# abelxiaoxing/ImageClassification

Hardware: AMD Instinct MI355X
Metric: images/sec (whole node) ResNet-50 bf16 224^2 training (higher is better)
Workload: dtype bf16; 1 GPU; resnet50 train step, synthetic 3x224x224, batch 256/GPU, AdamW, label smoothing 0.1, 1000 classes (BASELINE configs[1]); global_batch=256, parallelism=dp1

## Files before the change

imageclassification_amd/csrc/capi.hip:

```cpp
#include "capi_common.h"

bool g_prof_on = false;
std::vector<ProfRec> g_prof_recs;
std::vector<hipEvent_t> g_prof_pool;
hipEvent_t prof_event() {
  if (!g_prof_pool.empty()) { hipEvent_t e = g_prof_pool.back(); g_prof_pool.pop_back(); return e; }
  hipEvent_t e; (void)hipEventCreate(&e); return e;
}

extern "C" {

int icamd_abi_version(void) { return 6; }

int icamd_prof_enable(int on) { g_prof_on = on != 0; return ICAMD_OK; }
int icamd_prof_classes(void) { return PC_COUNT; }
int icamd_prof_collect(double* ms, long long* calls, double* bytes, double* flops, int n) {
  if (ms == nullptr || calls == nullptr || n < PC_COUNT) return ICAMD_ERR_BAD_ARG;
  for (auto& r : g_prof_recs) {
    (void)hipEventSynchronize(r.b);
    float t = 0.f;
    (void)hipEventElapsedTime(&t, r.a, r.b);
    ms[r.cls] += (double)t;
    calls[r.cls] += 1;
    if (bytes != nullptr) bytes[r.cls] += r.bytes;
    if (flops != nullptr) flops[r.cls] += r.flops;
    g_prof_pool.push_back(r.a);
    g_prof_pool.push_back(r.b);
  }
  g_prof_recs.clear();
  return ICAMD_OK;
}

int icamd_conv2d_stats_rows(const icamd_conv_desc* d) {
  if (!conv_desc_ok(d)) return 0;
  const long long M = (long long)d->N * d->OH * d->OW;
  return (int)((M + 127) / 128);
}

static int conv_fwd_impl(const icamd_conv_desc* d, const void* x, const void* w, void* y, const float* bias,
                         const void* addend, float* stats, int relu, void* stream, void* gelu_out = nullptr,
                         int gelu_inplace = 0) {
  if (!conv_desc_ok(d) || x == nullptr || w == nullptr || y == nullptr) return ICAMD_ERR_BAD_ARG;
  if ((long long)d->N * d->OH * d->OW >= (1ll << 31)) return ICAMD_ERR_UNSUPPORTED;
  if (d->KH == 3 && d->KW == 3 && d->stride == 1 && d->pad == 1 && addend == nullptr && gelu_out == nullptr &&
      !gelu_inplace && icamd_halo3x3_wanted(d->N, d->IH, d->IW, d->Cin, d->Cout)) {
    Halo3x3Params h;
    memset(&h, 0, sizeof(h));
    h.in = (const bf16_t*)x; h.wt = (const bf16_t*)w; h.out = (bf16_t*)y; h.bias = bias; h.stats = stats; h.relu = relu;
    h.N = d->N; h.H = d->IH; h.W = d->IW; h.C = d->Cin; h.Cout = d->Cout;
    return icamd_halo3x3_launch(h, (hipStream_t)stream);
  }
  const bool pw_gather = d->KH == 1 && d->KW == 1 && d->stride == 2 && d->pad == 0 && addend == nullptr;
  if (d->KH == 1 && d->KW == 1 && (d->stride == 1 || pw_gather) && d->pad == 0 && bias == nullptr && addend == nullptr && !relu &&
      gelu_out == nullptr && !gelu_inplace && icamd_pw_resident_wanted((long long)d->N * d->OH * d->OW, d->Cout, d->Cin)) {
    PwResidentParams g;
    memset(&g, 0, sizeof(g));
    g.A = (const bf16_t*)x; g.B = (const bf16_t*)w; g.out = (bf16_t*)y; g.stats = stats;
    g.M = d->N * d->OH * d->OW; g.N = d->Cout; g.K = d->Cin;
    if (pw_gather) { g.gat_oh = d->OH; g.gat_ow = d->OW; g.gat_ih = d->IH; g.gat_iw = d->IW; }
    return icamd_pw_resident_launch(g, (hipStream_t)stream);
  }
  if (d->KH == 1 && d->KW == 1 && (d->stride == 1 || pw_gather) && d->pad == 0 && (bias != nullptr || relu) && stats == nullptr &&
      gelu_out == nullptr && !gelu_inplace &&
      icamd_pw_resident_wanted((long long)d->N * d->OH * d->OW, d->Cout, d->Cin, addend != nullptr)) {
    PwResidentParams g;
    memset(&g, 0, sizeof(g));
    g.A = (const bf16_t*)x; g.B = (const bf16_t*)w; g.out = (bf16_t*)y; g.bias = bias; g.relu = relu;
    g.addend = (const bf16_t*)addend;
    g.M = d->N * d->OH * d->OW; g.N = d->Cout; g.K = d->Cin;
    if (pw_gather) { g.gat_oh = d->OH; g.gat_ow = d->OW; g.gat_ih = d->IH; g.gat_iw = d->IW; }
    return icamd_pw_resident_launch(g, (hipStream_t)stream);
  }
  if (d->KH == 1 && d->KW == 1 && d->stride == 1 && d->pad == 0 && addend == nullptr && !relu && stats == nullptr &&
      icamd_pw_resident_ext_wanted((long long)d->N * d->OH * d->OW, d->Cout, d->Cin)) {
    PwResidentParams g;
    memset(&g, 0, sizeof(g));
    g.A = (const bf16_t*)x; g.B = (const bf16_t*)w; g.out = (bf16_t*)y; g.bias = bias;
    g.gelu_out = (bf16_t*)gelu_out; g.gelu_inplace = gelu_inplace;
    g.M = d->N * d->OH * d->OW; g.N = d->Cout; g.K = d->Cin;
    return icamd_pw_resident_ext_launch(g, (hipStream_t)stream);
  }
  if (d->KH == 1 && d->KW == 1 && d->stride == 1 && d->pad == 0 &&
      icamd_gemm_nt_wanted((long long)d->N * d->OH * d->OW, d->Cout, d->Cin)) {
    GemmNtParams g;
    memset(&g, 0, sizeof(g));
    g.A = (const bf16_t*)x; g.B = (const bf16_t*)w; g.out = (bf16_t*)y; g.addend = (const bf16_t*)addend; g.bias = bias;
    g.stats = stats;
    g.M = d->N * d->OH * d->OW; g.N = d->Cout; g.K = d->Cin; g.relu = relu; g.gelu_out = (bf16_t*)gelu_out; g.gelu_inplace = gelu_inplace;
    return icamd_gemm_nt_launch(g, (hipStream_t)stream);
  }
  IgemmParams p;
  memset(&p, 0, sizeof(p));
  p.in = (const bf16_t*)x; p.wt = (const bf16_t*)w; p.out = (bf16_t*)y;
  p.addend = (const bf16_t*)addend; p.bias = bias; p.stats = stats; p.relu = relu; p.gelu_out = (bf16_t*)gelu_out; p.gelu_inplace = gelu_inplace;
  p.N = d->N; p.IH = d->IH; p.IW = d->IW; p.Cin = d->Cin;
  p.OH = d->OH; p.OW = d->OW; p.Cout = d->Cout;
  p.P = d->OH; p.Q = d->OW; p.M = d->N * d->OH * d->OW;
  p.ostr = 1; p.ooff_h = 0; p.ooff_w = 0; p.istr = d->stride;
  p.ntaps = d->KH * d->KW; p.Ktot = p.ntaps * d->Cin;
  p.KW = d->KW; p.pad = d->pad; p.tap_sign = 1; p.regular_taps = 1;
  if (p.ntaps <= ICAMD_MAX_TAPS)
    for (int r = 0; r < d->KH; ++r)
      for (int s = 0; s < d->KW; ++s) {
        const int t = r * d->KW + s;
        p.dh[t] = (short)(r - d->pad); p.dw[t] = (short)(s - d->pad); p.wtap[t] = (short)t;
      }
  return icamd_igemm_launch(p, (hipStream_t)stream);
}

int icamd_conv2d_fwd(const icamd_conv_desc* d, const void* x, const void* w, void* y, const float* bias,
                     const void* addend, float* stats, void* stream) {
  ProfScope _prof(PC_IGEMM_FWD, stream);
  const ConvWork cw = conv_work(d); _prof.work(cw.in + cw.out + 2 * cw.w + (addend ? cw.out : 0), cw.flops);
  return conv_fwd_impl(d, x, w, y, bias, addend, stats, 0, stream);
}

int icamd_conv2d_fwd_act(const icamd_conv_desc* d, const void* x, const void* w, void* y, const float* bias,
                         const void* addend, int relu, void* stream) {
  ProfScope _prof(PC_IGEMM_FWD, stream);
  const ConvWork cw = conv_work(d); _prof.work(cw.in + cw.out + 2 * cw.w + (addend ? cw.out : 0), cw.flops);
  return conv_fwd_impl(d, x, w, y, bias, addend, nullptr, relu ? 1 : 0, stream);
}

int icamd_conv2d_fwd_gelu(const icamd_conv_desc* d, const void* x, const void* w, void* z, void* a, const float* bias,
                          void* stream) {
  ProfScope _prof(PC_IGEMM_FWD, stream);
  const ConvWork cw = conv_work(d); _prof.work(cw.in + (z ? cw.out : 0) + cw.out + 2 * cw.w, cw.flops);
  if (a == nullptr) return ICAMD_ERR_BAD_ARG;
  if (z == nullptr) return conv_fwd_impl(d, x, w, a, bias, nullptr, nullptr, 0, stream, nullptr, 1);
  return conv_fwd_impl(d, x, w, z, bias, nullptr, nullptr, 0, stream, a);
}

static int dgrad_impl(const icamd_conv_desc* d, const void* dy, const void* w_t, void* dx, const void* addend,
                      const uint8_t* addend_bits, const icamd_bn_bwd_fuse* f, void* stream, const void* gelu_z = nullptr,
                      int addend_sub2 = 0) {
  if (!conv_desc_ok(d) || dy == nullptr || w_t == nullptr || dx == nullptr) return ICAMD_ERR_BAD_ARG;
  if (d->Cout % 8 != 0 || d->Cin % 8 != 0) return ICAMD_ERR_UNSUPPORTED;
  if ((long long)d->N * d->IH * d->IW >= (1ll << 31)) return ICAMD_ERR_UNSUPPORTED;
  const int st = d->stride;
  const bool pw_addend = icamd_pw_resident_mode() != 5;
  if (d->KH == 1 && d->KW == 1 && st == 1 && d->pad == 0 && f == nullptr && gelu_z == nullptr &&
      (addend == nullptr || pw_addend) && !(addend_bits != nullptr && addend_sub2) &&
      icamd_pw_resident_wanted((long long)d->N * d->IH * d->IW, d->Cin, d->Cout, addend != nullptr)) {
    PwResidentParams g;
    memset(&g, 0, sizeof(g));
    g.A = (const bf16_t*)dy; g.B = (const bf16_t*)w_t; g.out = (bf16_t*)dx; g.addend = (const bf16_t*)addend;
    g.addend_bits = addend_bits;
    g.M = d->N * d->IH * d->IW; g.N = d->Cin; g.K = d->Cout;
    if (addend_sub2) { g.sub2_h = d->IH; g.sub2_w = d->IW; }
    return icamd_pw_resident_launch(g, (hipStream_t)stream);
  }
  if (d->KH == 1 && d->KW == 1 && st == 1 && d->pad == 0 && f == nullptr && addend == nullptr &&
      icamd_pw_resident_ext_wanted((long long)d->N * d->IH * d->IW, d->Cin, d->Cout)) {
    PwResidentParams g;
    memset(&g, 0, sizeof(g));
    g.A = (const bf16_t*)dy; g.B = (const bf16_t*)w_t; g.out = (bf16_t*)dx; g.gelu_z = (const bf16_t*)gelu_z;
    g.M = d->N * d->IH * d->IW; g.N = d->Cin; g.K = d->Cout;
    return icamd_pw_resident_ext_launch(g, (hipStream_t)stream);
  }
  if (d->KH == 1 && d->KW == 1 && st == 1 && d->pad == 0 && f == nullptr && !(addend_bits != nullptr && addend_sub2) &&
      icamd_gemm_nt_wanted((long long)d->N * d->IH * d->IW, d->Cin, d->Cout)) {
    GemmNtParams g;
    memset(&g, 0, sizeof(g));
    g.A = (const bf16_t*)dy; g.B = (const bf16_t*)w_t; g.out = (bf16_t*)dx; g.addend = (const bf16_t*)addend;
    g.addend_bits = addend_bits;
    g.M = d->N * d->IH * d->IW; g.N = d->Cin; g.K = d->Cout; g.gelu_z = (const bf16_t*)gelu_z;
    if (addend_sub2) { g.sub2_h = d->IH; g.sub2_w = d->IW; }
    return icamd_gemm_nt_launch(g, (hipStream_t)stream);
  }
  if (d->KH == 3 && d->KW == 3 && st == 1 && d->pad == 1 && addend == nullptr && addend_bits == nullptr && f == nullptr &&
      gelu_z == nullptr && icamd_halo3x3_wanted(d->N, d->IH, d->IW, d->Cout, d->Cin)) {
    Halo3x3Params h;
    memset(&h, 0, sizeof(h));
    h.in = (const bf16_t*)dy; h.wt = (const bf16_t*)w_t; h.out = (bf16_t*)dx; h.flip = 1;
    h.N = d->N; h.H = d->IH; h.W = d->IW; h.C = d->Cout; h.Cout = d->Cin;
    return icamd_halo3x3_launch(h, (hipStream_t)stream);
  }
  float* partials = f ? f->partials : nullptr;
  for (int ph = 0; ph < st; ++ph)
    for (int pw = 0; pw < st; ++pw) {
      const int P = (d->IH - ph + st - 1) / st, Q = (d->IW - pw + st - 1) / st;
      if (P <= 0 || Q <= 0) continue;
      IgemmParams p;
      memset(&p, 0, sizeof(p));
      p.in = (const bf16_t*)dy; p.wt = (const bf16_t*)w_t; p.out = (bf16_t*)dx;
      p.addend = (const bf16_t*)addend;
      p.addend_bits = addend_bits;
      p.addend_sub2 = addend_sub2;
      p.gelu_z = (const bf16_t*)gelu_z;
      p.N = d->N; p.IH = d->OH; p.IW = d->OW; p.Cin = d->Cout;
      p.OH = d->IH; p.OW = d->IW; p.Cout = d->Cin;
      p.P = P; p.Q = Q; p.M = d->N * P * Q;
      p.ostr = st; p.ooff_h = ph; p.ooff_w = pw; p.istr = 1;
      p.Ktot = d->KH * d->KW * d->Cout;
      p.KW = d->KW; p.pad = d->pad; p.tap_sign = -1; p.regular_taps = (st == 1) ? 1 : 0;
      if (f != nullptr) {
        p.bnb_y = (const bf16_t*)f->y; p.bnb_mask = (const bf16_t*)f->mask_src;
        p.bnb_mean = f->mean; p.bnb_invstd = f->invstd; p.bnb_scale = f->scale; p.bnb_shift = f->shift;
        p.bnb_relu = f->relu; p.stats = partials;
        partials += (size_t)((p.M + 127) / 128) * 2 * d->Cin;
      }
      int nt = 0;
      for (int r = 0; r < d->KH; ++r) {
        const int eh = ph + d->pad - r;
        if (((eh % st) + st) % st != 0) continue;
        for (int s = 0; s < d->KW; ++s) {
          const int ew = pw + d->pad - s;
          if (((ew % st) + st) % st != 0) continue;
          if (nt < ICAMD_MAX_TAPS) { p.dh[nt] = (short)(eh / st); p.dw[nt] = (short)(ew / st); p.wtap[nt] = (short)(r * d->KW + s); }
          ++nt;
        }
      }
      p.ntaps = nt;
      const int rc = icamd_igemm_launch(p, (hipStream_t)stream);
      if (rc) return rc;
    }
  return ICAMD_OK;
}

int icamd_conv2d_dgrad(const icamd_conv_desc* d, const void* dy, const void* w_t, void* dx, const void* addend,
                       const uint8_t* addend_maskbits, void* stream) {
  ProfScope _prof(PC_IGEMM_DGRAD, stream);
  const ConvWork cw = conv_work(d); _prof.work(cw.out + cw.in + 2 * cw.w + (addend ? cw.in : 0) + (addend_maskbits ? cw.in / 16 : 0), cw.flops);
  if (addend_maskbits != nullptr && (addend == nullptr || d == nullptr || d->Cin % 64 != 0)) return ICAMD_ERR_BAD_ARG;
  return dgrad_impl(d, dy, w_t, dx, addend, addend_maskbits, nullptr, stream);
}

int icamd_conv2d_dgrad_sub2(const icamd_conv_desc* d, const void* dy, const void* w_t, void* dx, const void* addend_sub2,
                            void* stream) {
  ProfScope _prof(PC_IGEMM_DGRAD, stream);
  const ConvWork cw = conv_work(d); _prof.work(cw.out + cw.in + 2 * cw.w + cw.in / 4, cw.flops);
  if (addend_sub2 == nullptr) return ICAMD_ERR_BAD_ARG;
  return dgrad_impl(d, dy, w_t, dx, addend_sub2, nullptr, nullptr, stream, nullptr, 1);
}

int icamd_conv2d_dgrad_gelu(const icamd_conv_desc* d, const void* dy, const void* w_t, const void* z, void* dz,
                            void* stream) {
  ProfScope _prof(PC_IGEMM_DGRAD, stream);
  const ConvWork cw = conv_work(d); _prof.work(cw.out + 2 * cw.in + 2 * cw.w, cw.flops);
  if (z == nullptr) return ICAMD_ERR_BAD_ARG;
  return dgrad_impl(d, dy, w_t, dz, nullptr, nullptr, nullptr, stream, z);
}

int icamd_conv2d_dgrad_stats_rows(const icamd_conv_desc* d) {
  if (!conv_desc_ok(d)) return 0;
  int rows = 0;
  for (int ph = 0; ph < d->stride; ++ph)
    for (int pw = 0; pw < d->stride; ++pw) {
      const long long P = (d->IH - ph + d->stride - 1) / d->stride, Q = (d->IW - pw + d->stride - 1) / d->stride;
      if (P > 0 && Q > 0) rows += (int)((d->N * P * Q + 127) / 128);
    }
  return rows;
}

int icamd_conv2d_dgrad_bnbwd(const icamd_conv_desc* d, const void* dy, const void* w_t, void* g, const void* addend,
                             const icamd_bn_bwd_fuse* f, void* stream) {
  ProfScope _prof(PC_IGEMM_DGRAD, stream);
  const ConvWork cw = conv_work(d); _prof.work(cw.out + 2 * cw.in + 2 * cw.w + (addend ? cw.in : 0), cw.flops);
  if (f == nullptr || f->y == nullptr || f->mean == nullptr || f->invstd == nullptr || f->partials == nullptr)
// ... 89 lines not shown
```

imageclassification_amd/csrc/conv3x3_halo.hip:

```cpp
#ifndef ICAMD_C64_NT
#define ICAMD_C64_NT 0
#endif
#include "common.h"
#include "icamd_internal.h"
#include <cstdlib>

namespace {

template <int N> __device__ __forceinline__ void halo_wait_vmcnt() {
  static_assert(N >= 0 && N < 64, "vmcnt is a 6-bit field");
  asm volatile("s_waitcnt vmcnt(%0)" ::"n"(N) : "memory");
}

__device__ __forceinline__ int swzq(int blk) { return (0x78 >> (2 * blk)) & 3; }

template <int BN, int WN, int MFR, int LA, int NB, int KS, int WPS>
__global__ __launch_bounds__(256, WPS) void conv3x3_halo_kernel(const Halo3x3Params p) {
  constexpr int WM = 4 / WN;
  constexpr int BM = WM * MFR * 16;
  constexpr int NJ = BN / WN / 16;
  constexpr int A_SLOTS = 4 * LA * 8;
  constexpr int ZERO_SLOT = A_SLOTS - 1;
  constexpr int A_BYTES = A_SLOTS * 128;
  constexpr int B_STAGE = BN * KS * 2;
  constexpr int LB = BN * KS / 2048;
  static_assert(KS == 32 || KS == 64, "filter stage width");
  constexpr int RING = NB * B_STAGE;
  constexpr int EPI_BYTES = BM * BN * 2;
  constexpr int LDS_BYTES = (A_BYTES + RING > EPI_BYTES) ? A_BYTES + RING : EPI_BYTES;
  static_assert(NB >= 2 && NB <= 8 && (WN == 1 || WN == 2) && LB >= 1, "configuration");
  __shared__ __attribute__((aligned(16))) unsigned char smem[LDS_BYTES];
  unsigned char* const sA = smem;
  unsigned char* const sB = smem + A_BYTES;

  const int tid = threadIdx.x, lane = tid & 63;
  const int wave = __builtin_amdgcn_readfirstlane(tid >> 6);
  const int wm = wave % WM, wn = wave / WM;
  const int fr = lane & 15, fq = lane >> 4;

  const unsigned int nblk = gridDim.x;
  unsigned int L;
  {
    const unsigned int xcd = blockIdx.x & 7u, idx = blockIdx.x >> 3;
    const unsigned int q = nblk >> 3, r = nblk & 7u;
    L = (xcd < r ? xcd * (q + 1) : r * (q + 1) + (xcd - r) * q) + idx;
  }
  const int tile_m = L / p.ntiles_n, tile_n = L - tile_m * p.ntiles_n;
  const int m0 = tile_m * BM, n0 = tile_n * BN;
  const int W = p.W, C = p.C;
  const bf16_t* __restrict__ in = p.in;
  const bf16_t* __restrict__ wt = p.wt;
  const bf16_t* zero = (const bf16_t*)icamd_zero_page;

  const int a_slot_lane = lane >> 3;
  int b_src[LB];
#pragma unroll
  for (int j = 0; j < LB; ++j) {
    int row, lc;
    if constexpr (KS == 64) {
      row = (wave * LB + j) * 8 + (lane >> 3);
      lc = ((lane & 7) ^ ((row >> 1) & 7)) * 8;
    } else {
      row = (wave * LB + j) * 16 + (lane >> 2);
      lc = ((lane & 3) ^ swzq((row >> 2) & 3)) * 8;
    }
    const int co = n0 + row;
    b_src[j] = (co < p.Cout) ? co * 9 * C + lc : -1;
  }
  auto stage_a = [&](int slice) {
#pragma unroll
    for (int j = 0; j < LA; ++j) {
      const int slot = (wave * LA + j) * 8 + a_slot_lane;
      const int pix = m0 - (W + 1) + slot;
      const int lc = (((lane & 7) - slot) & 7) * 8;
      const bf16_t* src = (pix >= 0 && pix < p.M && slot != ZERO_SLOT) ? in + ((long long)pix * C + slice * 64 + lc) : zero;
      __builtin_amdgcn_global_load_lds(GPTR(src), LPTR(sA + (wave * LA + j) * 1024), 16, 0, 0);
    }
  };
  auto stage_b = [&](int slice, int tap, int kk, int slot) {
    const int wtap = p.flip ? 8 - tap : tap;
    const int off = wtap * C + slice * 64 + kk * 32;
#pragma unroll
    for (int j = 0; j < LB; ++j) {
      const bf16_t* src = b_src[j] >= 0 ? wt + (b_src[j] + off) : zero;
      __builtin_amdgcn_global_load_lds(GPTR(src), LPTR(sB + slot * B_STAGE + (wave * LB + j) * 1024), 16, 0, 0);
    }
  };

  int slot0[MFR];
  unsigned int vmask[MFR];
#pragma unroll
  for (int i = 0; i < MFR; ++i) {
    const int ml = wm * (BM / WM) + i * 16 + fr;
    const int m = m0 + ml;
    slot0[i] = ml + W + 1;
    unsigned int mk = 0;
    if (m < p.M) {
      const unsigned int n = fdiv((unsigned)m, p.divHW);
      const unsigned int rem = m - n * (p.H * W);
      const int h = (int)fdiv(rem, p.divW);
      const int w = (int)(rem - (unsigned)h * W);
#pragma unroll
      for (int t = 0; t < 9; ++t) {
        const int dh = t / 3 - 1, dw = t % 3 - 1;
        if ((unsigned)(h + dh) < (unsigned)p.H && (unsigned)(w + dw) < (unsigned)W) mk |= 1u << t;
      }
    }
    vmask[i] = mk;
  }
  f32x4 acc[NJ][MFR];
#pragma unroll
  for (int j = 0; j < NJ; ++j)
#pragma unroll
    for (int i = 0; i < MFR; ++i) acc[j][i] = f32x4{0.f, 0.f, 0.f, 0.f};

  const int nslices = C >> 6;
  constexpr int SPT = 64 / KS;
  const int nstages = nslices * 9 * SPT;
  stage_a(0);
  int issue_q = 0, issue_slice = 0, issue_tap = 0, issue_kk = 0, fill = 0;
  auto issue_b = [&]() {
    stage_b(issue_slice, issue_tap, issue_kk, fill);
    fill = fill == NB - 1 ? 0 : fill + 1;
    ++issue_q;
    if (++issue_kk == SPT) {
      issue_kk = 0;
      if (++issue_tap == 9) { issue_tap = 0; ++issue_slice; }
    }
  };
#pragma unroll
  for (int k = 0; k < NB - 1; ++k)
    if (issue_q < nstages) issue_b();

  const int b_row = wn * (BN / WN) + fr;
  const int b_frag = KS == 64 ? b_row * 128 : b_row * 64 + ((fq ^ swzq((fr >> 2) & 3)) << 4);
  const int bsw = (fr >> 1) & 7;
  int read = 0, q = 0;
  for (int slice = 0; slice < nslices; ++slice) {
#pragma unroll 1
    for (int tap = 0; tap < 9; ++tap) {
      const int trow = tap >= 6 ? 2 : (tap >= 3 ? 1 : 0);
      const int doff = (trow - 1) * W + (tap - 3 * trow - 1);
      const unsigned int tbit = 1u << tap;
      int aaddr[MFR];
#pragma unroll
      for (int i = 0; i < MFR; ++i) {
        const int sl = (vmask[i] & tbit) ? slot0[i] + doff : ZERO_SLOT;
        aaddr[i] = sl * 128 + (((fq + sl) & 7) << 4);
      }
#pragma unroll
      for (int st = 0; st < SPT; ++st, ++q) {
        {
          const int younger = issue_q - 1 - q;
          if (younger >= 4) halo_wait_vmcnt<4 * LB>();
          else if (younger == 3) halo_wait_vmcnt<3 * LB>();
          else if (younger == 2) halo_wait_vmcnt<2 * LB>();
          else if (younger == 1) halo_wait_vmcnt<LB>();
          else halo_wait_vmcnt<0>();
        }
        asm volatile("s_waitcnt lgkmcnt(0)" ::: "memory");
        __builtin_amdgcn_s_barrier();
        if (issue_q < nstages) issue_b();
        const unsigned char* sb = sB + read * B_STAGE + b_frag;
        read = read == NB - 1 ? 0 : read + 1;
#pragma unroll
        for (int kk = (KS == 64 ? 0 : st); kk < (KS == 64 ? 2 : st + 1); ++kk) {
          bf16x8 wf[NJ];
#pragma unroll
          for (int j = 0; j < NJ; ++j) {
            if constexpr (KS == 64) wf[j] = *(const bf16x8*)(sb + j * 2048 + (((kk * 4 + fq) ^ bsw) << 4));
            else wf[j] = *(const bf16x8*)(sb + j * 1024);
          }
#pragma unroll
          for (int i = 0; i < MFR; ++i) {
            const bf16x8 xf = *(const bf16x8*)(sA + (kk ? (aaddr[i] ^ 64) : aaddr[i]));
#pragma unroll
            for (int j = 0; j < NJ; ++j) acc[j][i] = __builtin_amdgcn_mfma_f32_16x16x32_bf16(wf[j], xf, acc[j][i], 0, 0, 0);
          }
        }
      }
    }
    if (slice + 1 < nslices) {
      asm volatile("s_waitcnt lgkmcnt(0)" ::: "memory");
      __builtin_amdgcn_s_barrier();
      stage_a(slice + 1);
      halo_wait_vmcnt<0>();
    }
  }
  __syncthreads();

  constexpr int ROWB = BN * 2, CPR = BN / 8;
#pragma unroll
  for (int j = 0; j < NJ; ++j) {
    const int cl = wn * (BN / WN) + j * 16 + 4 * fq;
    const int cg = n0 + cl;
    const int cgc = cg < p.Cout ? cg : 0;
    f32x4 b4 = {0.f, 0.f, 0.f, 0.f};
    if (p.bias != nullptr) b4 = *(const f32x4*)(p.bias + cgc);
#pragma unroll
    for (int i = 0; i < MFR; ++i) {
      const int ml = wm * (BM / WM) + i * 16 + fr;
      f32x4 v = acc[j][i] + b4;
      if (p.relu) {
#pragma unroll
        for (int e = 0; e < 4; ++e) v[e] = v[e] < 0.f ? 0.f : v[e];
      }
      u32x2 pk;
      pk[0] = pack_bf16x2(v[0], v[1]);
      pk[1] = pack_bf16x2(v[2], v[3]);
      const int slot = cl >> 2;
      *(u32x2*)(smem + ml * ROWB + ((((slot >> 1) ^ ml) & (CPR - 1)) << 4) + ((slot & 1) << 3)) = pk;
    }
  }
  __syncthreads();
  constexpr int RPP = 256 / CPR;
  constexpr int NPASS = BM / RPP;
  const int cp = tid & (CPR - 1), rg = tid / CPR;
  const int co = n0 + cp * 8;
  const bool co_ok = co < p.Cout;
  float s1[8], s2[8];
#pragma unroll
  for (int e = 0; e < 8; ++e) { s1[e] = 0.f; s2[e] = 0.f; }
#pragma unroll
  for (int ps = 0; ps < NPASS; ++ps) {
    const int ml = ps * RPP + rg;
    const int m = m0 + ml;
    const u32x4 o = *(const u32x4*)(smem + ml * ROWB + (((cp ^ ml) & (CPR - 1)) << 4));
    if (m < p.M && co_ok) {
      *(u32x4*)(p.out + (long long)m * p.Cout + co) = o;
      if (p.stats != nullptr) {
#pragma unroll
        for (int e = 0; e < 4; ++e) {
          const float lo = bf16_lo(o[e]), hi = bf16_hi(o[e]);
          s1[2 * e] += lo; s2[2 * e] += lo * lo;
          s1[2 * e + 1] += hi; s2[2 * e + 1] += hi * hi;
        }
      }
    }
  }
  if (p.stats != nullptr) {
    __syncthreads();
    float* red = (float*)smem;
#pragma unroll
    for (int e = 0; e < 8; ++e) {
      red[(rg * 2 + 0) * BN + cp * 8 + e] = s1[e];
      red[(rg * 2 + 1) * BN + cp * 8 + e] = s2[e];
    }
    __syncthreads();
    const int ntm = (p.M + BM - 1) / BM, nrows = (p.M + 127) / 128;
    for (int idx = tid; idx < 2 * BN; idx += 256) {
      const int which = idx / BN, c = idx - which * BN;
      float s = 0.f;
#pragma unroll 4
      for (int g = 0; g < RPP; ++g) s += red[(g * 2 + which) * BN + c];
      if (n0 + c < p.Cout) {
        p.stats[((long long)tile_m * 2 + which) * p.Cout + n0 + c] = s;
        if (ntm + tile_m < nrows) p.stats[((long long)(ntm + tile_m) * 2 + which) * p.Cout + n0 + c] = 0.f;
      }
    }
  }
}

template <bool ACT>
__global__ __launch_bounds__(256, 2) void conv3x3_c64_resident_kernel(const Halo3x3Params p, const int ntiles) {
  constexpr int BM = 128, LA = 8;
  constexpr int A_BYTES = 32 * LA * 128;
  constexpr int E_BYTES = 4 * 64 * 64;
  constexpr int ZERO_SLOT = 32 * LA - 1;
  __shared__ __attribute__((aligned(16))) unsigned char smem[2 * A_BYTES + E_BYTES];

  const int tid = threadIdx.x, lane = tid & 63;
  const int wave = __builtin_amdgcn_readfirstlane(tid >> 6);
  const int wm = wave & 1, wn = wave >> 1;
  const int fr = lane & 15, fq = lane >> 4;
  const int W = p.W, H = p.H;
  const bf16_t* __restrict__ in = p.in;
  const bf16_t* zero = (const bf16_t*)icamd_zero_page;
  unsigned char* const sE = smem + 2 * A_BYTES + wave * 4096;
  const unsigned lds_base = (unsigned)(uintptr_t)LPTR(smem);

  const int a_slot = wave * 8 + (lane >> 3);
  const int a_lc = (((lane & 7) - (lane >> 3)) & 7) * 8;
  const bool a_zero_lane = a_slot == 31;
  auto stage_a = [&](int m0, unsigned char* dst) {
    const int pix0 = m0 - (W + 1) + a_slot;
    const bf16_t* src0 = in + ((long long)pix0 * 64 + a_lc);
    if (m0 - (W + 1) >= 0 && m0 - (W + 1) + LA * 32 <= p.M) {
#pragma unroll
      for (int j = 0; j < LA; ++j) {
        const bf16_t* src = src0 + j * (32 * 64);
        if (j == LA - 1) src = a_zero_lane ? zero : src;
        __builtin_amdgcn_global_load_lds(GPTR(src), LPTR(dst + (j * 4 + wave) * 1024), 16, 0, ICAMD_C64_NT);
      }
    } else {
#pragma unroll
      for (int j = 0; j < LA; ++j) {
        const int pix = pix0 + j * 32;
        const bf16_t* src = (pix >= 0 && pix < p.M && !(j == LA - 1 && a_zero_lane)) ? src0 + j * (32 * 64) : zero;
        __builtin_amdgcn_global_load_lds(GPTR(src), LPTR(dst + (j * 4 + wave) * 1024), 16, 0, ICAMD_C64_NT);
      }
    }
  };

  int buf = 0;
  int tile = blockIdx.x;
  if (tile < ntiles) stage_a(tile * BM, smem);

  bf16x8 wf[18][2];
#pragma unroll
  for (int ks = 0; ks < 18; ++ks) {
    const int tap = ks >> 1;
// ... 93 lines not shown
      for (int i = 0; i < 4; ++i) {
        const int pl = i * 16 + fr;
        f32x4 v = acc[j][i];
        if constexpr (ACT) {
          v += b4;
          if (p.relu) {
#pragma unroll
            for (int e = 0; e < 4; ++e) v[e] = v[e] < 0.f ? 0.f : v[e];
          }
        }
        u32x2 pk;
        pk[0] = pack_bf16x2(v[0], v[1]);
        pk[1] = pack_bf16x2(v[2], v[3]);
        const int slot = j * 4 + fq;
        *(u32x2*)(sE + pl * 64 + ((((slot >> 1) ^ (pl >> 2)) & 3) << 4) + ((slot & 1) << 3)) = pk;
      }
    }
    {
      const int pl0 = lane >> 2;
      const int mrow = m0 + wm * 64 + pl0;
      bf16_t* orow = p.out + ((long long)mrow * 64 + wn * 32 + (lane & 3) * 8);
      const bool want_stats = p.stats != nullptr;
#pragma unroll
      for (int r = 0; r < 4; ++r) {
        const int pl = r * 16 + pl0;
        const u32x4 o = *(const u32x4*)(sE + pl * 64 + ((((lane & 3) ^ (pl >> 2)) & 3) << 4));
        if (mrow + r * 16 < p.M) {
          *(u32x4*)(orow + r * (16 * 64)) = o;
          if (want_stats) {
#pragma unroll
            for (int e = 0; e < 4; ++e) {
              const f32x2 v = {bf16_lo(o[e]), bf16_hi(o[e])};
              s1[e] += v;
              s2[e] = __builtin_elementwise_fma(v, v, s2[e]);
            }
          }
        }
      }
    }
  }

  if (p.stats != nullptr) {
    __syncthreads();
    float* red = (float*)smem;
    const int g = wm * 16 + (lane >> 2);
    const int c0 = wn * 32 + (lane & 3) * 8;
#pragma unroll
    for (int e = 0; e < 4; ++e) {
      red[(g * 2 + 0) * 64 + c0 + 2 * e] = s1[e][0];
      red[(g * 2 + 0) * 64 + c0 + 2 * e + 1] = s1[e][1];
      red[(g * 2 + 1) * 64 + c0 + 2 * e] = s2[e][0];
      red[(g * 2 + 1) * 64 + c0 + 2 * e + 1] = s2[e][1];
    }
    __syncthreads();
    if (tid < 128) {
      const int which = tid >> 6, c = tid & 63;
      float s = 0.f;
#pragma unroll 8
      for (int k = 0; k < 32; ++k) s += red[(k * 2 + which) * 64 + c];
      p.stats[((long long)blockIdx.x * 2 + which) * 64 + c] = s;
      const int nrows = (p.M + 127) / 128;
      for (int r = blockIdx.x + gridDim.x; r < nrows; r += gridDim.x) p.stats[((long long)r * 2 + which) * 64 + c] = 0.f;
    }
  }
}

int launch_resident_c64(const Halo3x3Params& p, hipStream_t stream) {
  const int ntiles = (p.M + 127) / 128;
  const int slots = 2 * icamd_num_cus();
  const int grid = ntiles < slots ? ntiles : slots;
  if (p.bias != nullptr || p.relu)
    hipLaunchKernelGGL((conv3x3_c64_resident_kernel<true>), dim3((unsigned)grid), dim3(256), 0, stream, p, ntiles);
  else
    hipLaunchKernelGGL((conv3x3_c64_resident_kernel<false>), dim3((unsigned)grid), dim3(256), 0, stream, p, ntiles);
  return icamd_launch_status();
}

template <int BN, int WN, int MFR, int LA, int NB, int KS, int WPS>
int launch_halo(const Halo3x3Params& p, hipStream_t stream) {
  constexpr int BM = (4 / WN) * MFR * 16;
  const int ntm = (p.M + BM - 1) / BM;
  hipLaunchKernelGGL((conv3x3_halo_kernel<BN, WN, MFR, LA, NB, KS, WPS>), dim3((unsigned)(ntm * p.ntiles_n)), dim3(256), 0,
                     stream, p);
  return icamd_launch_status();
}

int halo_mode() {
  static const int m = icamd_env_int("ICAMD_CONV3X3_HALO", 1);
  return m;
}

}

static bool resident_c64_ok(int W, int C, int Cout) {
  static const int on = icamd_env_int("ICAMD_CONV3X3_RESIDENT", 1);
  return on != 0 && C == 64 && Cout == 64 && W % 8 == 0 && 128 + 2 * W + 2 <= 255;
}

bool icamd_halo3x3_wanted(int N, int H, int W, int C, int Cout) {
  if (halo_mode() == 0) return false;
  if (C % 64 != 0 || Cout % 8 != 0 || W < 3 || H < 3) return false;
  if (resident_c64_ok(W, C, Cout)) return true;
  if (halo_mode() == 1 && C < 256) return false;
  if ((long long)N * H * W >= (1ll << 30)) return false;
  if (2 * W + 3 + 128 > 4 * 8 * 8) return false;
  return true;
}

int icamd_halo3x3_launch(Halo3x3Params& p, hipStream_t stream) {
  if (!icamd_halo3x3_wanted(p.N, p.H, p.W, p.C, p.Cout)) return ICAMD_ERR_UNSUPPORTED;
  p.M = p.N * p.H * p.W;
  p.divHW = make_fastdiv((unsigned)(p.H * p.W));
  p.divW = make_fastdiv((unsigned)p.W);
  if (resident_c64_ok(p.W, p.C, p.Cout)) return launch_resident_c64(p, stream);
  const int bn = p.Cout <= 64 ? 64 : 128;
  p.ntiles_n = (p.Cout + bn - 1) / bn;
  int bm = 128;
  if (halo_mode() == 3) bm = 256;
  else if (halo_mode() != 2) {
    long long best = -1;
    for (int cand : {256, 224, 128}) {
      if (cand == 224 && bn != 128) continue;
      if ((cand + 2 * p.W + 3 + 31) / 32 > (cand == 128 ? 8 : 12)) continue;
      const long long tiles = (long long)((p.M + cand - 1) / cand) * p.ntiles_n;
      const long long cost = ((tiles + 511) / 512) * cand + (cand == 128 ? 16 : 0);
      if (best < 0 || cost < best) { best = cost; bm = cand; }
    }
  }
  const bool big = bm != 128;
  const int slots = bm + 2 * p.W + 2 + 1;
  const int la = (slots + 31) / 32;
  if (la > 12) return ICAMD_ERR_UNSUPPORTED;
  if (bn == 128) {
    if (bm == 224) {
      if (la <= 8) return launch_halo<128, 2, 7, 8, 3, 64, 2>(p, stream);
      if (la <= 10) return launch_halo<128, 2, 7, 10, 2, 64, 2>(p, stream);
      return launch_halo<128, 2, 7, 12, 2, 64, 2>(p, stream);
    }
    if (big) {
      if (la <= 9) return launch_halo<128, 2, 8, 9, 2, 64, 2>(p, stream);
      if (la <= 10) return launch_halo<128, 2, 8, 10, 2, 64, 2>(p, stream);
      return launch_halo<128, 2, 8, 12, 2, 64, 2>(p, stream);
    }
    if (la <= 5) return launch_halo<128, 2, 4, 5, 3, 64, 2>(p, stream);
    if (la <= 6) return launch_halo<128, 2, 4, 6, 3, 64, 2>(p, stream);
    return launch_halo<128, 2, 4, 8, 3, 64, 2>(p, stream);
  }
  if (big) {
    if (la <= 9) return launch_halo<64, 1, 4, 9, 6, 32, 2>(p, stream);
    if (la <= 10) return launch_halo<64, 1, 4, 10, 6, 32, 2>(p, stream);
    return launch_halo<64, 1, 4, 12, 6, 32, 2>(p, stream);
  }
  if (la <= 5) return launch_halo<64, 1, 2, 5, 6, 32, 3>(p, stream);
  if (la <= 6) return launch_halo<64, 1, 2, 6, 6, 32, 3>(p, stream);
  return launch_halo<64, 1, 2, 8, 6, 32, 2>(p, stream);
}
```

imageclassification_amd/csrc/icamd_internal.h:

```cpp
#pragma once
#include "common.h"

#define ICAMD_MAX_TAPS 56

struct IgemmParams {
  const bf16_t* in;
  const bf16_t* wt;
  bf16_t* out;
  const bf16_t* addend;
  const unsigned char* addend_bits;
  int addend_sub2;
  const float* bias;
  float* stats;
  const bf16_t* bnb_y;
  const bf16_t* bnb_mask;
  const float *bnb_mean, *bnb_invstd, *bnb_scale, *bnb_shift;
  int bnb_relu;
  int relu;
  bf16_t* gelu_out;
  int gelu_inplace;
  const bf16_t* gelu_z;
  int N, IH, IW, Cin;
  int OH, OW, Cout;
  int P, Q, M;
  int ostr, ooff_h, ooff_w, istr;
  int ntaps, Ktot;
  int KW, pad;
  int tap_sign, regular_taps;
  int stem7;
  int ksteps, ntiles_n;
  FastDiv divPQ, divQ, divCin, divKW;
  short dh[ICAMD_MAX_TAPS], dw[ICAMD_MAX_TAPS], wtap[ICAMD_MAX_TAPS];
};
int icamd_igemm_launch(IgemmParams& p, hipStream_t stream);
int icamd_igemm_pick_bn(int Cout);

struct Halo3x3Params {
  const bf16_t* in;
  const bf16_t* wt;
  bf16_t* out;
  const float* bias;
  float* stats;
  int relu;
  int flip;
  int N, H, W, C, Cout;
  int M, ntiles_n;
  FastDiv divHW, divW;
};
bool icamd_halo3x3_wanted(int N, int H, int W, int C, int Cout);
int icamd_halo3x3_launch(Halo3x3Params& p, hipStream_t stream);

struct GConvParams {
  const bf16_t* in;
  const bf16_t* w;
  bf16_t* out;
  const bf16_t* dy;
  float* slab;
  const float* bias;
  float* stats;
  int relu;
  int N, IH, IW, OH, OW, C, groups, stride;
  int Cg, M, npix_in, nalloc;
  int S, tiles_per_split, ntiles;
  FastDiv divOHW, divOW;
};
bool icamd_gconv3x3_ok(int N, int IH, int IW, int OH, int OW, int C, int groups, int stride);
int icamd_gconv3x3_fwd_launch(GConvParams& p, hipStream_t stream);
int icamd_gconv3x3_dgrad_launch(GConvParams& p, hipStream_t stream);
size_t icamd_gconv3x3_wgrad_bytes(int N, int IH, int IW, int OH, int OW, int C, int groups, int stride);
int icamd_gconv3x3_wgrad_launch(GConvParams& p, hipStream_t stream);

struct Pool2x2Params {
  const bf16_t* in;
  const bf16_t* addend;
  bf16_t* out;
  int N, IH, IW, C8;
  int OH, OW;
  unsigned int total;
  FastDiv divC8, divOW, divOH;
};
bool icamd_avgpool2x2_ok(int N, int IH, int IW, int C);
int icamd_avgpool2x2_launch(Pool2x2Params& p, int backward, hipStream_t stream);

struct ThinConvParams {
  const bf16_t* in;
  const bf16_t* w;
  bf16_t* out;
  const bf16_t* dy;
  float* slab;
  const float* bias;
  float* stats;
  int relu;
  int N, H, W, Cout;
  int M, nalloc, ntiles;
  int S, tiles_per_split;
  FastDiv divHW, divW;
};
bool icamd_thin3x3_ok(int N, int H, int W, int Cin, int Cout);
int icamd_thin3x3_stats_rows(int N, int H, int W, int Cout);
int icamd_thin3x3_fwd_launch(ThinConvParams& p, hipStream_t stream);
int icamd_thin3x3_dgrad_launch(ThinConvParams& p, hipStream_t stream);
size_t icamd_thin3x3_wgrad_bytes(int N, int H, int W, int Cout);
int icamd_thin3x3_wgrad_launch(ThinConvParams& p, hipStream_t stream);

struct GemmNtParams {
  const bf16_t* A;
  const bf16_t* B;
  bf16_t* out;
  const bf16_t* addend;
  const unsigned char* addend_bits;
  const float* bias;
  float* stats;
  int M, N, K;
  int sub2_h, sub2_w;
  FastDiv divHW, divW;
  int relu;
  bf16_t* gelu_out;
  int gelu_inplace;
  const bf16_t* gelu_z;
  int ntiles_n;
  int group_n;
  int out_policy;
};
int icamd_gemm_nt_launch(GemmNtParams& p, hipStream_t stream);
bool icamd_gemm_nt_wanted(long long M, int N, int K);

struct PwResidentParams {
  const bf16_t* A;
  const bf16_t* B;
  bf16_t* out;
  const bf16_t* addend;
  const unsigned char* addend_bits;
  float* stats;
// ... 247 lines not shown
```

Baseline: 14760 images/sec.

## Add halo-tiled stride-2 3x3 conv kernels for forward and dgrad

Extends the halo 3x3 conv kernel with two stride-2 modes. The forward mode restages the input halo per parity sub-grid of the input. The dgrad mode splits the output into four parity classes, each running only its contributing taps and scattering the results. These replace the generic implicit-GEMM path for large-channel stride-2 3x3 convs, to cut redundant gathers and work on zero taps. The cost is extra barriers and restaging in the forward mode, and scattered writes in dgrad.

```diff
diff --git a/imageclassification_amd/csrc/capi.hip b/imageclassification_amd/csrc/capi.hip
--- a/imageclassification_amd/csrc/capi.hip
+++ b/imageclassification_amd/csrc/capi.hip
@@ -49,6 +49,14 @@
     h.in = (const bf16_t*)x; h.wt = (const bf16_t*)w; h.out = (bf16_t*)y; h.bias = bias; h.stats = stats; h.relu = relu;
     h.N = d->N; h.H = d->IH; h.W = d->IW; h.C = d->Cin; h.Cout = d->Cout;
     return icamd_halo3x3_launch(h, (hipStream_t)stream);
+  }
+  if (d->KH == 3 && d->KW == 3 && d->stride == 2 && d->pad == 1 && addend == nullptr && gelu_out == nullptr &&
+      !gelu_inplace && icamd_halo3x3_s2_wanted(d->N, d->IH, d->IW, d->Cin, d->Cout, false)) {
+    Halo3x3Params h;
+    memset(&h, 0, sizeof(h));
+    h.in = (const bf16_t*)x; h.wt = (const bf16_t*)w; h.out = (bf16_t*)y; h.bias = bias; h.stats = stats; h.relu = relu;
+    h.N = d->N; h.FH = d->IH; h.FW = d->IW; h.C = d->Cin; h.Cout = d->Cout;
+    return icamd_halo3x3_s2_launch(h, false, (hipStream_t)stream);
   }
   const bool pw_gather = d->KH == 1 && d->KW == 1 && d->stride == 2 && d->pad == 0 && addend == nullptr;
   if (d->KH == 1 && d->KW == 1 && (d->stride == 1 || pw_gather) && d->pad == 0 && bias == nullptr && addend == nullptr && !relu &&
@@ -175,6 +183,14 @@
     h.in = (const bf16_t*)dy; h.wt = (const bf16_t*)w_t; h.out = (bf16_t*)dx; h.flip = 1;
     h.N = d->N; h.H = d->IH; h.W = d->IW; h.C = d->Cout; h.Cout = d->Cin;
     return icamd_halo3x3_launch(h, (hipStream_t)stream);
+  }
+  if (d->KH == 3 && d->KW == 3 && st == 2 && d->pad == 1 && addend == nullptr && addend_bits == nullptr && f == nullptr &&
+      gelu_z == nullptr && icamd_halo3x3_s2_wanted(d->N, d->IH, d->IW, d->Cout, d->Cin, true)) {
+    Halo3x3Params h;
+    memset(&h, 0, sizeof(h));
+    h.in = (const bf16_t*)dy; h.wt = (const bf16_t*)w_t; h.out = (bf16_t*)dx;
+    h.N = d->N; h.FH = d->IH; h.FW = d->IW; h.C = d->Cout; h.Cout = d->Cin;
+    return icamd_halo3x3_s2_launch(h, true, (hipStream_t)stream);
   }
   float* partials = f ? f->partials : nullptr;
   for (int ph = 0; ph < st; ++ph)
diff --git a/imageclassification_amd/csrc/conv3x3_halo.hip b/imageclassification_amd/csrc/conv3x3_halo.hip
--- a/imageclassification_amd/csrc/conv3x3_halo.hip
+++ b/imageclassification_amd/csrc/conv3x3_halo.hip
@@ -3,6 +3,7 @@
 #endif
 #include "common.h"
 #include "icamd_internal.h"
+#include "conv3x3_s2_taps.h"
 #include <cstdlib>
 
 namespace {
@@ -14,7 +15,7 @@
 
 __device__ __forceinline__ int swzq(int blk) { return (0x78 >> (2 * blk)) & 3; }
 
-template <int BN, int WN, int MFR, int LA, int NB, int KS, int WPS>
+template <int BN, int WN, int MFR, int LA, int NB, int KS, int WPS, int MODE = 0>
 __global__ __launch_bounds__(256, WPS) void conv3x3_halo_kernel(const Halo3x3Params p) {
   constexpr int WM = 4 / WN;
   constexpr int BM = WM * MFR * 16;
@@ -45,8 +46,22 @@
     const unsigned int q = nblk >> 3, r = nblk & 7u;
     L = (xcd < r ? xcd * (q + 1) : r * (q + 1) + (xcd - r) * q) + idx;
   }
-  const int tile_m = L / p.ntiles_n, tile_n = L - tile_m * p.ntiles_n;
+  int tile_m, tile_n, cls = 3;
+  if constexpr (MODE == 2) {
+    const int per_m = 4 * p.ntiles_n;
+    tile_m = L / per_m;
+    const int rem = L - tile_m * per_m;
+    const int rank = rem / p.ntiles_n;
+    tile_n = rem - rank * p.ntiles_n;
+    cls = 3 - rank;
+  } else {
+    tile_m = L / p.ntiles_n;
+    tile_n = L - tile_m * p.ntiles_n;
+  }
   const int m0 = tile_m * BM, n0 = tile_n * BN;
+  const int ntap = MODE == 2 ? icamd_s2_class_ntaps(cls) : 9;
+  const unsigned long long tapseq = MODE == 2 ? kS2TapSeq >> (4 * icamd_s2_class_first(cls)) : kS2TapSeq;
+  constexpr int ABASE = MODE == 2 ? 0 : 1;
   const int W = p.W, C = p.C;
   const bf16_t* __restrict__ in = p.in;
   const bf16_t* __restrict__ wt = p.wt;
@@ -67,18 +82,46 @@
     const int co = n0 + row;
     b_src[j] = (co < p.Cout) ? co * 9 * C + lc : -1;
   }
-  auto stage_a = [&](int slice) {
+  [[maybe_unused]] int s2_pix[MODE == 1 ? LA : 1];
+  unsigned long long s2_ok = 0;
+  if constexpr (MODE == 1) {
 #pragma unroll
     for (int j = 0; j < LA; ++j) {
       const int slot = (wave * LA + j) * 8 + a_slot_lane;
-      const int pix = m0 - (W + 1) + slot;
+      const int g = m0 - (W + 1) + slot;
+      s2_pix[j] = 0;
+      if (g >= 0 && g < p.M && slot < p.nslots) {
+        const unsigned int n = fdiv((unsigned)g, p.divHW);
+        const unsigned int rem = g - n * (p.H * W);
+        const int a = (int)fdiv(rem, p.divW);
+        const int b = (int)(rem - (unsigned)a * W);
+        s2_pix[j] = ((int)n * p.FH + 2 * a) * p.FW + 2 * b;
+        const unsigned int okh = 2 * a + 1 < p.FH, okw = 2 * b + 1 < p.FW;
+        s2_ok |= (unsigned long long)(1u | (okw << 1) | (okh << 2) | ((okh & okw) << 3)) << (4 * j);
+      }
+    }
+  }
+  auto stage_a = [&](int slice, int sub) {
+#pragma unroll
+    for (int j = 0; j < LA; ++j) {
+      const int slot = (wave * LA + j) * 8 + a_slot_lane;
       const int lc = (((lane & 7) - slot) & 7) * 8;
-      const bf16_t* src = (pix >= 0 && pix < p.M && slot != ZERO_SLOT) ? in + ((long long)pix * C + slice * 64 + lc) : zero;
+      const bf16_t* src;
+      if constexpr (MODE == 0) {
+        const int pix = m0 - (W + 1) + slot;
+        src = (pix >= 0 && pix < p.M && slot != ZERO_SLOT) ? in + ((long long)pix * C + slice * 64 + lc) : zero;
+      } else if constexpr (MODE == 1) {
+        const int pix = s2_pix[j] + (sub >> 1) * p.FW + (sub & 1);
+        src = ((s2_ok >> (4 * j + sub)) & 1) ? in + ((long long)pix * C + slice * 64 + lc) : zero;
+      } else {
+        const int pix = m0 + slot;
+        src = (pix < p.M && slot < p.nslots) ? in + ((long long)pix * C + slice * 64 + lc) : zero;
+      }
       __builtin_amdgcn_global_load_lds(GPTR(src), LPTR(sA + (wave * LA + j) * 1024), 16, 0, 0);
     }
   };
   auto stage_b = [&](int slice, int tap, int kk, int slot) {
-    const int wtap = p.flip ? 8 - tap : tap;
+    const int wtap = MODE != 0 ? (int)((tapseq >> (4 * tap)) & 15) : (p.flip ? 8 - tap : tap);
     const int off = wtap * C + slice * 64 + kk * 32;
 #pragma unroll
     for (int j = 0; j < LB; ++j) {
@@ -93,7 +136,7 @@
   for (int i = 0; i < MFR; ++i) {
     const int ml = wm * (BM / WM) + i * 16 + fr;
     const int m = m0 + ml;
-    slot0[i] = ml + W + 1;
+    slot0[i] = ml + ABASE * (W + 1);
     unsigned int mk = 0;
     if (m < p.M) {
       const unsigned int n = fdiv((unsigned)m, p.divHW);
@@ -102,7 +145,8 @@
       const int w = (int)(rem - (unsigned)h * W);
 #pragma unroll
       for (int t = 0; t < 9; ++t) {
-        const int dh = t / 3 - 1, dw = t % 3 - 1;
+        const int dh = MODE == 0 ? t / 3 - 1 : (MODE == 1 ? icamd_s2_fwd_off(t / 3) : icamd_s2_dgrad_off(t / 3));
+        const int dw = MODE == 0 ? t % 3 - 1 : (MODE == 1 ? icamd_s2_fwd_off(t % 3) : icamd_s2_dgrad_off(t % 3));
         if ((unsigned)(h + dh) < (unsigned)p.H && (unsigned)(w + dw) < (unsigned)W) mk |= 1u << t;
       }
     }
@@ -116,8 +160,8 @@
 
   const int nslices = C >> 6;
   constexpr int SPT = 64 / KS;
-  const int nstages = nslices * 9 * SPT;
-  stage_a(0);
+  const int nstages = nslices * ntap * SPT;
+  stage_a(0, 3);
   int issue_q = 0, issue_slice = 0, issue_tap = 0, issue_kk = 0, fill = 0;
   auto issue_b = [&]() {
     stage_b(issue_slice, issue_tap, issue_kk, fill);
@@ -125,7 +169,7 @@
     ++issue_q;
     if (++issue_kk == SPT) {
       issue_kk = 0;
-      if (++issue_tap == 9) { issue_tap = 0; ++issue_slice; }
+      if (++issue_tap == ntap) { issue_tap = 0; ++issue_slice; }
     }
   };
 #pragma unroll
@@ -138,10 +182,28 @@
   int read = 0, q = 0;
   for (int slice = 0; slice < nslices; ++slice) {
 #pragma unroll 1
-    for (int tap = 0; tap < 9; ++tap) {
-      const int trow = tap >= 6 ? 2 : (tap >= 3 ? 1 : 0);
-      const int doff = (trow - 1) * W + (tap - 3 * trow - 1);
-      const unsigned int tbit = 1u << tap;
+    for (int tap = 0; tap < ntap; ++tap) {
+      int doff;
+      unsigned int tbit;
+      if constexpr (MODE == 0) {
+        const int trow = tap >= 6 ? 2 : (tap >= 3 ? 1 : 0);
+        doff = (trow - 1) * W + (tap - 3 * trow - 1);
+        tbit = 1u << tap;
+      } else {
+        const int wtap = (int)((tapseq >> (4 * tap)) & 15);
+        const int trow = wtap >= 6 ? 2 : (wtap >= 3 ? 1 : 0);
+        const int near_h = trow == 0, near_w = wtap - 3 * trow == 0;
+        doff = MODE == 1 ? -(near_h * W + near_w) : near_h * W + near_w;
+        tbit = 1u << wtap;
+        if constexpr (MODE == 1) {
+          if (tap == 4 || tap == 6 || tap == 8) {
+            asm volatile("s_waitcnt lgkmcnt(0)" ::: "memory");
+            __builtin_amdgcn_s_barrier();
+            stage_a(slice, tap == 4 ? 2 : (tap == 6 ? 1 : 0));
+            halo_wait_vmcnt<0>();
+          }
+        }
+      }
       int aaddr[MFR];
 #pragma unroll
       for (int i = 0; i < MFR; ++i) {
@@ -183,7 +245,7 @@
     if (slice + 1 < nslices) {
       asm volatile("s_waitcnt lgkmcnt(0)" ::: "memory");
       __builtin_amdgcn_s_barrier();
-      stage_a(slice + 1);
+      stage_a(slice + 1, 3);
       halo_wait_vmcnt<0>();
     }
   }
@@ -226,7 +288,16 @@
     const int ml = ps * RPP + rg;
     const int m = m0 + ml;
     const u32x4 o = *(const u32x4*)(smem + ml * ROWB + (((cp ^ ml) & (CPR - 1)) << 4));
-    if (m < p.M && co_ok) {
+    if constexpr (MODE == 2) {
+      if (m < p.M && co_ok) {
+        const unsigned int n = fdiv((unsigned)m, p.divHW);
+        const unsigned int rem = m - n * (p.H * W);
+        const int h = (int)fdiv(rem, p.divW);
+        const int w = (int)(rem - (unsigned)h * W);
+        const int oh = 2 * h + (cls >> 1), ow = 2 * w + (cls & 1);
+        if (oh < p.FH && ow < p.FW) *(u32x4*)(p.out + ((long long)((int)n * p.FH + oh) * p.FW + ow) * p.Cout + co) = o;
+      }
+    } else if (m < p.M && co_ok) {
       *(u32x4*)(p.out + (long long)m * p.Cout + co) = o;
       if (p.stats != nullptr) {
 #pragma unroll
@@ -486,6 +557,15 @@
   const int ntm = (p.M + BM - 1) / BM;
   hipLaunchKernelGGL((conv3x3_halo_kernel<BN, WN, MFR, LA, NB, KS, WPS>), dim3((unsigned)(ntm * p.ntiles_n)), dim3(256), 0,
                      stream, p);
+  return icamd_launch_status();
+}
+
+template <int MODE, int MFR, int LA, int NB, int WPS = 2>
+int launch_halo_s2(const Halo3x3Params& p, hipStream_t stream) {
+  constexpr int BM = 2 * MFR * 16;
+  const int ntm = (p.M + BM - 1) / BM;
+  const int nblk = ntm * p.ntiles_n * (MODE == 2 ? 4 : 1);
+  hipLaunchKernelGGL((conv3x3_halo_kernel<128, 2, MFR, LA, NB, 64, WPS, MODE>), dim3((unsigned)nblk), dim3(256), 0, stream, p);
   return icamd_launch_status();
 }
 
@@ -559,3 +639,49 @@
   if (la <= 6) return launch_halo<64, 1, 2, 6, 6, 32, 3>(p, stream);
   return launch_halo<64, 1, 2, 8, 6, 32, 2>(p, stream);
 }
+
+bool icamd_halo3x3_s2_wanted(int N, int IH, int IW, int C, int Cout, bool dgrad) {
+  if (halo_mode() == 0) return false;
+  if (C % 64 != 0 || Cout % 8 != 0 || IH < 3 || IW < 3) return false;
+  const int OH = (IH - 1) / 2 + 1, OW = (IW - 1) / 2 + 1;
+  if ((long long)N * IH * IW >= (1ll << 31) || (long long)N * OH * OW >= (1ll << 30)) return false;
+  if (128 + OW + 2 > 6 * 32) return false;
+  if (halo_mode() == 1 && (C < (dgrad ? 256 : 512) || Cout < 128)) return false;
+  return true;
+}
+
+int icamd_halo3x3_s2_launch(Halo3x3Params& p, bool dgrad, hipStream_t stream) {
+  if (!icamd_halo3x3_s2_wanted(p.N, p.FH, p.FW, p.C, p.Cout, dgrad)) return ICAMD_ERR_UNSUPPORTED;
+  p.H = (p.FH - 1) / 2 + 1;
+  p.W = (p.FW - 1) / 2 + 1;
+  p.M = p.N * p.H * p.W;
+  p.divHW = make_fastdiv((unsigned)(p.H * p.W));
+  p.divW = make_fastdiv((unsigned)p.W);
+  p.ntiles_n = (p.Cout + 127) / 128;
+  auto la_of = [&](int bm) { return (bm + p.W + 2 + 31) / 32; };
+  const int big = la_of(224) <= 8 ? 224 : 256;
+  int bm = 128;
+  if (halo_mode() == 3) bm = big;
+  else if (halo_mode() != 2) {
+    if (dgrad && la_of(128) <= 5) {
+      p.nslots = 128 + p.W + 1;
+      return launch_halo_s2<2, 4, 5, 2, 3>(p, stream);
+    }
+    long long best = -1;
+    for (int cand : {256, 224, 128}) {
+      if (la_of(cand) > (cand == 128 ? 6 : (cand == 224 ? 8 : 10))) continue;
+      const long long tiles = (long long)((p.M + cand - 1) / cand) * p.ntiles_n * (dgrad ? 4 : 1);
+      const long long cost = ((tiles + 511) / 512) * cand + (cand == 128 ? 16 : 0);
+      if (best < 0 || cost < best) { best = cost; bm = cand; }
+    }
+  }
+  p.nslots = bm + p.W + 1;
+  if (dgrad) {
+    if (bm == 224) return launch_halo_s2<2, 7, 8, 3>(p, stream);
+    if (bm == 256) return launch_halo_s2<2, 8, 10, 2>(p, stream);
+    return launch_halo_s2<2, 4, 6, 3>(p, stream);
+  }
+  if (bm == 224) return launch_halo_s2<1, 7, 8, 3>(p, stream);
+  if (bm == 256) return launch_halo_s2<1, 8, 10, 2>(p, stream);
+  return launch_halo_s2<1, 4, 6, 3>(p, stream);
+}
diff --git a/imageclassification_amd/csrc/conv3x3_s2_taps.h b/imageclassification_amd/csrc/conv3x3_s2_taps.h
--- /dev/null
+++ b/imageclassification_amd/csrc/conv3x3_s2_taps.h
@@ -0,0 +1,21 @@
+#pragma once
+
+constexpr int kS2TapOrder[9] = {0, 2, 6, 8, 1, 7, 3, 5, 4};
+constexpr unsigned long long kS2TapSeq = 0x453718620ull;
+
+constexpr int icamd_s2_class_ntaps(int cls) { return (1 + (cls >> 1)) * (1 + (cls & 1)); }
+constexpr int icamd_s2_class_first(int cls) { return cls == 3 ? 0 : (cls == 2 ? 4 : (cls == 1 ? 6 : 8)); }
+constexpr int icamd_s2_tap_class(int tap) { return 2 * (tap / 3 != 1) + (tap % 3 != 1); }
+constexpr int icamd_s2_fwd_off(int r) { return r == 0 ? -1 : 0; }
+constexpr int icamd_s2_dgrad_off(int r) { return r == 0 ? 1 : 0; }
+constexpr int icamd_s2_class_extent(int IH, int ph) { return (IH - ph + 1) / 2; }
+
+constexpr bool icamd_s2_table_consistent() {
+  for (int i = 0; i < 9; ++i)
+    if ((int)((kS2TapSeq >> (4 * i)) & 15) != kS2TapOrder[i]) return false;
+  for (int cls = 0; cls < 4; ++cls)
+    for (int k = 0; k < icamd_s2_class_ntaps(cls); ++k)
+      if (icamd_s2_tap_class(kS2TapOrder[icamd_s2_class_first(cls) + k]) != cls) return false;
+  return true;
+}
+static_assert(icamd_s2_table_consistent(), "tap order, packed tap order and class ranges must agree");
diff --git a/imageclassification_amd/csrc/icamd_internal.h b/imageclassification_amd/csrc/icamd_internal.h
--- a/imageclassification_amd/csrc/icamd_internal.h
+++ b/imageclassification_amd/csrc/icamd_internal.h
@@ -46,9 +46,13 @@
   int N, H, W, C, Cout;
   int M, ntiles_n;
   FastDiv divHW, divW;
+  int FH, FW;
+  int nslots;
 };
 bool icamd_halo3x3_wanted(int N, int H, int W, int C, int Cout);
 int icamd_halo3x3_launch(Halo3x3Params& p, hipStream_t stream);
+bool icamd_halo3x3_s2_wanted(int N, int IH, int IW, int C, int Cout, bool dgrad);
+int icamd_halo3x3_s2_launch(Halo3x3Params& p, bool dgrad, hipStream_t stream);
 
 struct GConvParams {
   const bf16_t* in;
```

New measurement: 14840 images/sec (median of 6 runs). No clear change (+0.5%).
